# theo2021/OnDA

Hardware: AMD Instinct MI355X
Metric: adaptation-step images/sec (fwd+bwd+proto) 512x1024 bs=4 (higher is better)
Workload: dtype f32 (f16x2 split emulation); 1 GPU; hybrid_switch adaptation step (step + update_ema), 1024x512, bs=4 per micro-batch, 1 micro-batch(es) per GPU and optimizer step, dynamic branch, DeepLabV2-ResNet50 ProDA head, random-init weights; global_batch=4, parallelism=dp1, branch=dynamic, micro_batches_per_gpu=1, inputs=resident in HBM

## Files before the change

### include/onda_hip.h

```cpp
#ifndef ONDA_HIP_H
#define ONDA_HIP_H

#include <stdint.h>

#ifdef __cplusplus
extern "C" {
#endif

typedef void* onda_stream_t;

#define ONDA_OK 0
#define ONDA_EINVAL (-1)
#define ONDA_EALIGN (-2)

typedef struct OndaConv {
  int B, Hi, Wi, Cin;
  int Ho, Wo, Cout;
  int kh, kw, stride, dil, pad;
  int ldx;
  int ldy;
  int ldr;
  int out_os;
  int Hf, Wf;
  int relu;
// ... 89 lines not shown

typedef struct OndaBnSide {
  const float* x;
  const float* partials;
  int tiles, tile_rows;
  float *mean, *invstd, *xhat_amax;
  float *running_mean, *running_var;
  int64_t* nbt;
  float momentum;
  const float *gamma, *beta;
  void* dx;
  float* dx_amax;
} OndaBnSide;
int onda_bn_pair_fwd_l2(const OndaBnSide* a, const OndaBnSide* b, float eps, int relu, void* out, float* out_amax, int64_t M, int C,
                        uint8_t* relu_mask, int64_t split, int run_group, onda_stream_t s);
int64_t onda_bn_pair_bwd_l2_ws(int64_t M, int C);
int onda_bn_pair_bwd_l2(const float* dout, const uint8_t* relu_mask, const OndaBnSide* a, const OndaBnSide* b, float* ws, int64_t M,
                        int C, int relu, int64_t split, onda_stream_t s);
int onda_bn_pair_bwd_affine_l2(const float* dout, const uint8_t* relu_mask, const OndaBnSide* a, const OndaBnSide* b, float* ws,
                               int64_t M, int C, int relu, int64_t split, float* dgamma_a, float* dbeta_a, float* dgamma_b,
                               float* dbeta_b, onda_stream_t s);

int onda_conv_wgrad_l2_variant(int Cout, int Cin);
int64_t onda_conv2d_wgrad_l2_table_stride(const OndaConv* c);
int onda_conv2d_wgrad_l2_table(const OndaConv* c, int32_t* table, onda_stream_t s);
int onda_conv2d_wgrad_l2(const void* xl, int64_t xplane, const float* xamax, const void* dyl, int64_t dyplane, const float* dyamax,
                         float* slabs, int lddy, int splitk, const OndaConv* c, onda_stream_t s);

int onda_conv2d_wgrad(const float* x, const float* dy, float* slabs, int lddy, int splitk,
                      const OndaConv* c, onda_stream_t s);
int onda_wgrad_reduce(const float* slabs, float* dw, int splitk, int Cout, int taps, int Cin,
                      int Cout_real, int Cin_real, int flat_k, int accumulate, onda_stream_t s);

int onda_pack_weight_fwd(const float* w_oihw, float* dst, int Cout, int Cin, int taps, int Cout_pad, int Kp,
                         onda_stream_t s);
int onda_pack_weight_dgrad(const float* w_oihw, float* dst, int Cout, int Cin, int taps, int Cout_pad,
                           onda_stream_t s);

int onda_stem_im2col(const float* x_nchw, float* col, int B, int H, int W, int Ho, int Wo, int Kp, onda_stream_t s);

int onda_bn_finalize(const float* partials, int tiles, int C, int64_t count, float eps, float* mean, float* invstd,
                     float* running_mean, float* running_var, int64_t* num_batches_tracked, float momentum,
                     onda_stream_t s);
int onda_bn_stats(const float* x, int64_t M, int C, int ldx, float* partials, int* tiles_out, onda_stream_t s);
int onda_bn_apply(const float* x, const float* mean, const float* invstd, const float* gamma, const float* beta,
                  const float* residual, float* out, int64_t M, int C, int relu, float* amax, onda_stream_t s);
// ... 154 lines not shown
```

### onda_amd/_lib.py

```python
import ctypes
import os
from ctypes import POINTER, Structure, c_char_p, c_float, c_int, c_int64, c_void_p

HERE = os.path.dirname(os.path.abspath(__file__))
LIB_PATH = os.environ.get("ONDA_LIB_PATH") or os.path.join(HERE, "libonda_hip.so")

P = c_void_p
I, L, F = c_int, c_int64, c_float


class OndaConv(Structure):
    _fields_ = [(n, c_int) for n in ("B Hi Wi Cin Ho Wo Cout kh kw stride dil pad ldx ldy ldr out_os Hf Wf relu").split()] + \
               [("run_if", c_void_p), ("stat_split", c_int64), ("plain_schedule", c_int), ("pix_table", c_void_p),
                ("pix_stride", c_int64)]


class OndaSwitchCfg(Structure):
    _fields_ = [("limit", c_int), ("level_kind", c_int), ("use_exp", c_int), ("pad_", c_int), ("exp_const", ctypes.c_double),
                ("one_minus_exp_const", ctypes.c_double), ("taps_total", ctypes.c_double), ("gray_lo", ctypes.c_double),
                ("gray_hi", ctypes.c_double), ("dev_threshold", ctypes.c_double)]


class OndaLimbOut(Structure):
    _fields_ = [("out", c_void_p), ("out_plane", c_int64), ("out_bound", c_void_p), ("out_amax", c_void_p), ("kb", c_void_p),
# ... 41 lines not shown
    "onda_conv2d_fwd": (I, [P, P, P, P, P, P, P, P, POINTER(OndaConv), P]),
    "onda_absmax": (I, [P, L, I, I, P, P]),
    "onda_pack_weight_h2": (I, [P, P, I, I, I, I, I, I, I, P, P]),
    "onda_pack_weights_h2_multi": (I, [P, I, L, P]),
    "onda_pack_blocks": (I, [I, I, I]),
    "onda_split_h2": (I, [P, L, I, I, P, I, L, P, P]),
    "onda_stem_im2col_l2": (I, [P, P, P, L, I, I, I, I, I, I, P]),
    "onda_s2d_split_h2": (I, [P, I, I, I, I, I, I, F, P, P, P]),
    "onda_d2s_bwd": (I, [P, P, P, I, I, I, I, I, I, F, P, P, P]),
    "onda_debug_stamps": (None, [P]),
    "onda_conv2d_fwd_l2_limbs": (I, [P, L, P, P, P, P, P, P, P, P, P]),
    "onda_switch_state_doubles": (I, [I]),
    "onda_switch_max_window": (I, []),
    "onda_switch_step": (I, [P, P, P, I, P, POINTER(OndaSwitchCfg), P, P]),
    "onda_select_prior": (I, [P, P, F, P, F, P, L, P]),
    "onda_gate_scalar": (I, [P, P, P, P]),
    "onda_conv_l2_variant": (I, [L, I]),
    "onda_conv_l2_kernel_id": (I, [L, I, I, I]),
    "onda_conv_l2_tiles_m": (I, [L, I, I, I]),
    "onda_conv_l2_tiles_m_split": (I, [L, I, I, I, L, I, POINTER(c_int)]),
    "onda_conv_l2_live_fraction": (ctypes.c_double, [POINTER(OndaConv), I]),
    "onda_conv_wgrad_l2_live_fraction": (ctypes.c_double, [POINTER(OndaConv), I]),
    "onda_conv_wgrad_l2_variant": (I, [I, I]),
    "onda_conv2d_wgrad_l2_table_stride": (L, [POINTER(OndaConv)]),
    "onda_conv2d_wgrad_l2_table": (I, [POINTER(OndaConv), P, P]),
    "onda_conv2d_wgrad_l2": (I, [P, L, P, P, L, P, P, I, I, POINTER(OndaConv), P]),
    "onda_conv2d_fwd_l2": (I, [P, L, P, P, P, P, P, P, P, P, I, P, P, POINTER(OndaConv), P]),
    "onda_conv2d_taps_fwd_l2": (I, [P, P, P, P, P, P, P, P, P, P, P, POINTER(OndaConv), POINTER(c_int), I, P]),
    "onda_pack_sum_h2": (I, [POINTER(c_void_p), I, P, P, I, I, I, I, I, P, P]),
    "onda_bn_finalize_l2": (I, [P, I, I, L, F, P, P, P, P, P, F, P, P, P, I, P, P, L, I, I, P, I, P]),
    "onda_bn_apply_l2": (I, [P, P, P, P, P, P, L, P, P, L, P, L, I, I, P, L, P]),
    "onda_bn_bwd_l2_ws": (L, [L, I]),
    "onda_bn_train_l2": (I, [P, P, I, F, P, P, P, P, P, F, P, P, P, P, I, P, P, P, L, I, P, L, I, I, P]),
    "onda_bn_bwd_l2": (I, [P, P, L, P, P, P, P, P, P, L, P, P, P, L, I, I, P, L, I, P]),
    "onda_bn_bwd_affine_l2": (I, [P, P, L, P, P, P, P, P, P, L, P, P, P, L, I, I, P, L, I, P, P, P]),
    "onda_bn_pair_fwd_l2": (I, [POINTER(OndaBnSide), POINTER(OndaBnSide), F, I, P, P, L, I, P, L, I, P]),
    "onda_bn_pair_bwd_l2_ws": (L, [L, I]),
    "onda_bn_pair_bwd_l2": (I, [P, P, POINTER(OndaBnSide), POINTER(OndaBnSide), P, L, I, I, L, P]),
    "onda_bn_pair_bwd_affine_l2": (I, [P, P, POINTER(OndaBnSide), POINTER(OndaBnSide), P, L, I, I, L, P, P, P, P, P]),
    "onda_conv2d_wgrad": (I, [P, P, P, I, I, POINTER(OndaConv), P]),
    "onda_wgrad_reduce": (I, [P, P, I, I, I, I, I, I, I, I, P]),
    "onda_pack_weight_fwd": (I, [P, P, I, I, I, I, I, P]),
    "onda_pack_weight_dgrad": (I, [P, P, I, I, I, I, P]),
    "onda_stem_im2col": (I, [P, P, I, I, I, I, I, I, P]),
    "onda_bn_finalize": (I, [P, I, I, L, F, P, P, P, P, P, F, P]),
    "onda_bn_stats": (I, [P, L, I, I, P, POINTER(c_int), P]),
# ... 99 lines not shown
```

### onda_amd/csrc/conv_common.h

```cpp
#pragma once
#include "common.h"

struct ConvK {
  const float* x;
  const void* w;
  float* y;
  const float* scale;
  const float* shift;
  const float* res;
  float* stats;
  OndaConv c;
  int M, tilesM, tilesN, taps, kcper;
  float* ws;
  int tiles_dp;
  float* amax = nullptr;
  int skip_dead_taps = 1;
  int late_issue = 1;
  _Float16* yl = nullptr;
  long long yplane = 0;
  float* ybound = nullptr;
  const float* kb = nullptr;
  const float* xtrue = nullptr;
  const _Float16* resl = nullptr;
  long long resplane = 0;
  const float* res_amax = nullptr;
  const float* res_true = nullptr;
  unsigned long long* stamps = nullptr;
  int stats_rows = 2;
  long long x_total = 0;
};

struct WgradK {
  const float* x;
  const float* dy;
  float* slabs;
  OndaConv c;
  int M, lddy, splitk, mchunk, tilesN, tilesC, taps;
  long long x_total = 0, dy_total = 0;
  unsigned long long* stamps = nullptr;
  const int* pix = nullptr;
  long long pix_stride = 0;
};

constexpr int BK = 32;

template <class B>
__device__ __forceinline__ int xcd_band(B bid, int nblk) {
  const int q = nblk >> 3, r = nblk & 7, xcd = bid & 7;
  return (xcd < r ? xcd * (q + 1) : r * (q + 1) + (xcd - r) * q) + (bid >> 3);
}

struct SkItem {
  bool dp;
  int tile, k_begin, k_end;
};
struct SkTile {
  long long t0, t1;
};
struct StreamK {
  int KT, tiles_dp, G;
// ... 167 lines not shown
```

### onda_amd/csrc/conv_l2.hip

```cpp
#include "conv_common.h"
#include "limbs.h"

namespace {

typedef _Float16 f16x8 __attribute__((ext_vector_type(8)));
typedef _Float16 f16x4 __attribute__((ext_vector_type(4)));
typedef int i32x4 __attribute__((ext_vector_type(4)));

#define ZZ(i, jj) (((i) & 1) ? 3 - (jj) : (jj))

#define MFMA_SNAKE(MI, ACC, A, B)                                                                                       \
  _Pragma("unroll") for (int i = 0; i < (MI); ++i) _Pragma("unroll") for (int jj = 0; jj < 4; ++jj)                     \
      ACC[i][ZZ(i, jj)] = __builtin_amdgcn_mfma_f32_16x16x32_f16(A, B[ZZ(i, jj)], ACC[i][ZZ(i, jj)], 0, 0, 0)
#define FRAG_READ4(DST, P) \
  _Pragma("unroll") for (int j = 0; j < 4; ++j) DST = *reinterpret_cast<const f16x8*>((P) + j * 2048)
template <int MI>
__device__ __forceinline__ void acc_clear(f32x4 (&acc)[MI][4], f32x4 (&accx)[MI][4]) {
#pragma unroll
  for (int i = 0; i < MI; ++i)
#pragma unroll
    for (int j = 0; j < 4; ++j)
#pragma unroll
      for (int e = 0; e < 4; ++e) acc[i][j][e] = accx[i][j][e] = 0.f;
}
// ... 1296 lines not shown
      }
      *reinterpret_cast<f32x4*>(srow) = s1;
      *reinterpret_cast<f32x4*>(srow + c.Cout) = s2;
      if (SR == 4) {
        *reinterpret_cast<f32x4*>(srow + 2 * c.Cout) = mn;
        *reinterpret_cast<f32x4*>(srow + 3 * c.Cout) = mxv;
      }
    }
  }
}

template <int OFS = 0>
__device__ __forceinline__ f16x8 tr_read8(unsigned a0, unsigned a1) {
  u32x2 lo, hi;
  asm volatile("ds_read_b64_tr_b16 %0, %1 offset:%2" : "=v"(lo) : "v"(a0), "n"(OFS));
  asm volatile("ds_read_b64_tr_b16 %0, %1 offset:%2" : "=v"(hi) : "v"(a1), "n"(OFS));
  const u32x4 r = {lo[0], lo[1], hi[0], hi[1]};
  return __builtin_bit_cast(f16x8, r);
}
__device__ __forceinline__ void lds_wait(f16x8& a, f16x8& b, f16x8& c_, f16x8& d) {
  asm volatile("s_waitcnt lgkmcnt(0)" : "+v"(a), "+v"(b), "+v"(c_), "+v"(d));
}

template <int WM, int WN, int STAGES, int OCC, int MODE = 0>
__global__ __launch_bounds__(WM * WN * 64, OCC) void conv_wgrad_l2_kernel(const WgradK a, unsigned xplane, unsigned dyplane, unsigned x_bytes,
                                                                         unsigned dy_bytes, const float* __restrict__ xamax,
                                                                         const float* __restrict__ dyamax) {
  constexpr int NW = WM * WN;
  constexpr int SA = (64 * WM) / 128, SB = (64 * WN) / 128;
  static_assert(SA >= 1 && SB >= 1, "tiles are multiples of 128 channels");
  constexpr int SUB = 32 * 512;
  constexpr int A_BYTES = SA * SUB, STAGE = A_BYTES + SB * SUB;
  constexpr int GPW = 8 / NW;
  static_assert(GPW >= 1 && 8 % NW == 0, "8 pixel groups per K-step");
  constexpr int DPW = GPW * (SA + SB) * 2;
  constexpr bool STAGGER = NW == 8;
  constexpr int MAX_KT = 2048;
  __shared__ __attribute__((aligned(16))) unsigned char lds[STAGES * STAGE + MAX_KT * 2];

  const OndaConv& c = a.c;
  const int t = threadIdx.x, lane = t & 63, wave = __builtin_amdgcn_readfirstlane(t >> 6);
  const int wm = wave / WN, wn = wave % WN;
  const bool late = wave >= NW / 2;

  int bid = xcd_band(blockIdx.x, gridDim.x);
  const int tile_c = bid % a.tilesC;
  bid /= a.tilesC;
  const int tap = bid % a.taps;
  bid /= a.taps;
  const int tile_n = bid % a.tilesN;
  const int ks = bid / a.tilesN;
  const int n0 = tile_n * (64 * WM), c0 = tile_c * (64 * WN);
  const int mbeg = ks * a.mchunk;
  const int mend = min(a.M, mbeg + a.mchunk);
  const int KT = mend > mbeg ? (mend - mbeg + 31) / 32 : 0;
  const int rr = tap / c.kw, ss = tap - rr * c.kw;
  const int dh = rr * c.dil - c.pad, dw = ss * c.dil - c.pad;
  unsigned long long* stp = a.stamps != nullptr && t == 0 && blockIdx.x < 4096 ? a.stamps + (size_t)blockIdx.x * 8 : nullptr;
  if (stp) stp[0] = __builtin_amdgcn_s_memtime();
  constexpr unsigned PAST = 0x7FFFF000u;
  const int b_first = mbeg / (c.Ho * c.Wo);
  const long long x_at = (long long)b_first * c.Hi * c.Wi * c.ldx * 4, dy_at = (long long)mbeg * a.lddy * 4;
  const long long x_left = a.x_total - x_at;
  const long long dy_left = MODE == 1 ? (long long)(mend - mbeg) * a.lddy * 4 : a.dy_total - dy_at;
  const __amdgpu_buffer_rsrc_t rx = make_rsrc(reinterpret_cast<const char*>(a.x) + x_at, (unsigned)(x_left < PAST ? (x_left > 0 ? x_left : 0) : PAST));
  const __amdgpu_buffer_rsrc_t rdy = make_rsrc(reinterpret_cast<const char*>(a.dy) + dy_at, (unsigned)(dy_left < PAST ? (dy_left > 0 ? dy_left : 0) : PAST));
  const Scale2 sx = scale_of(xamax), sd = scale_of(dyamax);
  const float unscale_a = sx.inv, unscale_b = sd.inv;

  unsigned short* live_list = reinterpret_cast<unsigned short*>(lds + STAGES * STAGE);
  int nlive = 0;
  {
    unsigned char* flags = lds;
    for (int kt = t; kt < KT; kt += NW * 64) {
      const int m_first = mbeg + kt * 32, m_last = min(mend, m_first + 32) - 1;
      const int r_first = m_first / c.Wo, r_last = m_last / c.Wo;
      bool live = false;
      for (int r = r_first; r <= r_last; ++r) live |= (unsigned)((r % c.Ho) * c.stride + dh) < (unsigned)c.Hi;
      flags[kt] = live;
    }
    __syncthreads();
    for (int base = 0; base < KT; base += 64) {
      const bool f = base + lane < KT && flags[base + lane];
      const unsigned long long mask = __ballot(f);
      if (f) live_list[nlive + __popcll(mask & ((1ull << lane) - 1))] = (unsigned short)(base + lane);
      nlive += __popcll(mask);
    }
    __syncthreads();
  }
  auto live_at = [&](int i) -> int { return __builtin_amdgcn_readfirstlane((int)live_list[i]); };

  const int lam = lane >> 5, limb = (lane >> 4) & 1;
  unsigned ch_dy[GPW][2][SA], ch_x[GPW][2][SB];
#pragma unroll
  for (int d = 0; d < GPW; ++d)
#pragma unroll
    for (int h = 0; h < 2; ++h) {
      const int row = (wave * GPW + d) * 4 + 2 * h + lam;
      const int swz = ((row & 3) << 2) | ((row >> 2) & 3);
      const int ch = (lane & 15) ^ swz;
#pragma unroll
      for (int sI = 0; sI < SA; ++sI) {
        const int n = n0 + sI * 128 + ch * 8;
        ch_dy[d][h][sI] = n < c.Cout ? (unsigned)(limb_at(0, n, 0) + limb * LIMB2_OFS) * 2u : PAST;
      }
#pragma unroll
      for (int sI = 0; sI < SB; ++sI) {
        const int cc = c0 + sI * 128 + ch * 8;
        ch_x[d][h][sI] = cc < c.Cin ? (unsigned)(limb_at(0, cc, 0) + limb * LIMB2_OFS) * 2u : PAST;
      }
    }
  int p_m[GPW], p_wo[GPW], p_ho[GPW], p_b[GPW];
#pragma unroll
  for (int d = 0; d < GPW; ++d) {
    const int m = mbeg + (wave * GPW + d) * 4 + 2 * lam;
    p_m[d] = m;
    p_wo[d] = m % c.Wo;
    const int tq = m / c.Wo;
    p_ho[d] = tq % c.Ho;
    p_b[d] = tq / c.Ho - b_first;
  }
  int k_decoded = 0;
  unsigned pdy_s[GPW][2], px_s[GPW][2];
  int stage_s = 0;
  auto issue_part = [&](int h) {
#if defined(__HIP_DEVICE_COMPILE__)
#pragma unroll
    for (int d = 0; d < GPW; ++d) {
      const int grp = wave * GPW + d;
#pragma unroll
      for (int sI = 0; sI < SA; ++sI) {
        unsigned char* dst = lds + stage_s + sI * SUB + (grp * 2 + h) * 1024;
        const unsigned vo = pdy_s[d][h] + ch_dy[d][h][sI];
        __builtin_amdgcn_raw_ptr_buffer_load_lds(rdy, (__attribute__((address_space(3))) void*)dst, 16, vo, 0, 0, 0);
      }
#pragma unroll
      for (int sI = 0; sI < SB; ++sI) {
        unsigned char* dst = lds + stage_s + A_BYTES + sI * SUB + (grp * 2 + h) * 1024;
        const unsigned vo = px_s[d][h] + ch_x[d][h][sI];
        __builtin_amdgcn_raw_ptr_buffer_load_lds(rx, (__attribute__((address_space(3))) void*)dst, 16, vo, 0, 0, 0);
      }
    }
#else
    (void)h;
#endif
  };
  auto issue_addr = [&](int kt, int stage_off) {
    stage_s = stage_off;
    const int adv = (kt - k_decoded) * 32;
    k_decoded = kt;
#pragma unroll
    for (int d = 0; d < GPW; ++d) {
      p_m[d] += adv;
      p_wo[d] += adv;
      while (p_wo[d] >= c.Wo) {
        p_wo[d] -= c.Wo;
        if (++p_ho[d] == c.Ho) {
          p_ho[d] = 0;
          ++p_b[d];
        }
      }
      int m = p_m[d], wo = p_wo[d], ho = p_ho[d], b = p_b[d];
#pragma unroll
      for (int h = 0; h < 2; ++h) {
        unsigned pdy = OOB, px = OOB;
        if (m < mend) {
          pdy = (unsigned)(m - mbeg) * (unsigned)a.lddy * 4u;
          const int hi = ho * c.stride + dh, wi = wo * c.stride + dw;
          if ((unsigned)hi < (unsigned)c.Hi && (unsigned)wi < (unsigned)c.Wi) px = (unsigned)(((b * c.Hi + hi) * c.Wi + wi) * c.ldx) * 4u;
        }
        pdy_s[d][h] = pdy;
        px_s[d][h] = px;
        ++m;
        if (++wo == c.Wo) {
          wo = 0;
          if (++ho == c.Ho) {
            ho = 0;
            ++b;
          }
        }
      }
    }
  };
  auto issue = [&](int kt, int stage_off) {
    issue_addr(kt, stage_off);
    issue_part(0);
    issue_part(1);
  };

  unsigned fa[4][2], fb[4][2];
  {
    const int g = lane >> 4, q = (lane >> 2) & 3, pp = lane & 3;
#pragma unroll
    for (int h = 0; h < 2; ++h) {
      const int row = 8 * g + 4 * h + q;
      const int swz = ((row & 3) << 2) | ((row >> 2) & 3);
#pragma unroll
      for (int i = 0; i < 4; ++i) {
        const int cha = (wm & 1) * 8 + 2 * i + (pp >> 1), chb = (wn & 1) * 8 + 2 * i + (pp >> 1);
        fa[i][h] = (unsigned)((wm >> 1) * SUB + 512 * row + 16 * (cha ^ swz) + 8 * (pp & 1));
        fb[i][h] = (unsigned)(A_BYTES + (wn >> 1) * SUB + 512 * row + 16 * (chb ^ swz) + 8 * (pp & 1));
        asm volatile("" : "+v"(fa[i][h]), "+v"(fb[i][h]));
      }
    }
  }

  f32x4 acc[4][4], accx[4][4];
  acc_clear(acc, accx);
// ... 17 lines not shown
      issue_part(0);
      st_issue = st_issue + STAGE == STAGES * STAGE ? 0 : st_issue + STAGE;
      ++i_iss;
    }
  };
  auto issue_second_part = [&]() {
    if (second_part_due) issue_part(1);
    second_part_due = false;
  };
  auto wait_landed_half = [&](bool first_part_in_flight) {
    if (first_part_in_flight)
      asm volatile("s_waitcnt vmcnt(%0)" ::"n"(DPW / 2) : "memory");
    else
      asm volatile("s_waitcnt vmcnt(0)" ::: "memory");
  };
  auto wait_landed = [&](bool more_in_flight) {
    if (more_in_flight)
      asm volatile("s_waitcnt vmcnt(%0)" ::"n"(DPW) : "memory");
    else
      asm volatile("s_waitcnt vmcnt(0)" ::: "memory");
  };
  constexpr int AHEAD = STAGES >= 3 ? 2 : 1;
  static_assert(!STAGGER || STAGES >= 3, "the staggered halves need two steps in flight");
  if constexpr (MODE == 0) {
    if (i_iss < nlive) issue_next();
    if (AHEAD == 2 && i_iss < nlive) issue_next();
  }
  f16x8 af[4][2], bf[4], b1[4];
  const unsigned lds0 = (unsigned)(size_t)(__attribute__((address_space(3))) unsigned char*)lds;
  unsigned base;
  auto prepare = [&]() {
    base = lds0 + st_read;
    st_read = st_read + STAGE == STAGES * STAGE ? 0 : st_read + STAGE;
#pragma unroll
    for (int i = 0; i < 4; ++i) {
      const unsigned a0 = base + fa[i][0], a1 = base + fa[i][1];
      af[i][0] = tr_read8<0>(a0, a1);
      af[i][1] = tr_read8<256>(a0, a1);
    }
#pragma unroll
    for (int j = 0; j < 4; ++j) {
      const unsigned a0 = base + fb[j][0], a1 = base + fb[j][1];
      bf[j] = tr_read8<256>(a0, a1);
      if constexpr (STAGGER) b1[j] = tr_read8<0>(a0, a1);
    }
  };
  auto prepared = [&]() {
    lds_wait(af[0][0], af[1][0], af[2][0], af[3][0]);
    lds_wait(af[0][1], af[1][1], af[2][1], af[3][1]);
    lds_wait(bf[0], bf[1], bf[2], bf[3]);
    if constexpr (STAGGER) lds_wait(b1[0], b1[1], b1[2], b1[3]);
    __builtin_amdgcn_sched_barrier(0);
  };
  auto compute = [&]() {
    if constexpr (!STAGGER) {
#pragma unroll
      for (int j = 0; j < 4; ++j) b1[j] = tr_read8(base + fb[j][0], base + fb[j][1]);
    }
    MFMA_SNAKE(4, accx, af[i][0], bf);
    if constexpr (!STAGGER) lds_wait(b1[0], b1[1], b1[2], b1[3]);
    if constexpr (STAGGER) issue_second_part();
    __builtin_amdgcn_sched_barrier(0);
    MFMA_SNAKE(4, accx, af[i][1], b1);
    MFMA_SNAKE(4, acc, af[i][0], b1);
  };
  if constexpr (MODE >= 1) {
    static_assert(STAGGER && GPW == 1 && STAGES == 3, "the eight-wave tile");
    const unsigned lddy4 = (unsigned)a.lddy * 4u, ldx4 = (unsigned)c.ldx * 4u;
    unsigned dy_lane[2], x_lane[2];
#pragma unroll
    for (int h = 0; h < 2; ++h) {
      const unsigned pix = (unsigned)(wave * 4 + 2 * lam + h);
      dy_lane[h] = pix * lddy4;
      x_lane[h] = (pix + (unsigned)(mbeg - b_first * c.Ho * c.Wo)) * ldx4;
    }
    const int base_px = b_first * c.Hi * c.Wi;
    const i32x4* tab = MODE == 2 ? reinterpret_cast<const i32x4*>(a.pix + (size_t)tap * a.pix_stride + mbeg + wave * 4) : nullptr;
    i32x4 t_next = {-1, -1, -1, -1};
    auto offsets = [&](int kt, const i32x4& te, unsigned kill) {
#pragma unroll
      for (int h = 0; h < 2; ++h) {
        pdy_s[0][h] = (unsigned)kt * 32u * lddy4 + dy_lane[h] + kill;
        if constexpr (MODE == 1) {
          px_s[0][h] = (unsigned)kt * 32u * ldx4 + x_lane[h] + kill;
        } else {
          const int lo = te[h], hi = te[2 + h];
          const int e = lam ? hi : lo;
          px_s[0][h] = (e >= 0 ? __umul24((unsigned)(e - base_px), ldx4) : PAST) + kill;
        }
// ... 61 lines not shown
        __builtin_amdgcn_sched_group_barrier(0x008, 16, 0);
#pragma unroll
        for (int q = 0; q < 14; ++q) {
          __builtin_amdgcn_sched_group_barrier(0x008, 1, 0);
          __builtin_amdgcn_sched_group_barrier(0x002, 2, 0);
        }
#pragma unroll
        for (int q = 0; q < NI; ++q) {
          __builtin_amdgcn_sched_group_barrier(0x008, 2, 0);
          __builtin_amdgcn_sched_group_barrier(0x006, 2, 0);
          __builtin_amdgcn_sched_group_barrier(0x020, 1, 0);
        }
        __builtin_amdgcn_sched_group_barrier(0x008, 48 - 16 - 14 - 2 * NI, 0);
        __builtin_amdgcn_sched_barrier(0);
        entry_wait(t_after);
        kt_next = kt_after;
        t_next = t_after;
      }
      if (!late) __builtin_amdgcn_s_barrier();
      asm volatile("s_waitcnt vmcnt(0)" ::: "memory");
    }
  } else if constexpr (!STAGGER) {
    for (; i_cur < nlive; ++i_cur) {
      wait_landed(AHEAD == 2 && i_cur + 1 < nlive);
      __builtin_amdgcn_s_barrier();
      if (i_iss < nlive) issue_next();
      prepare();
      prepared();
      compute();
    }
  } else {
    if (late && nlive > 0) {
      wait_landed(nlive > 1);
      __builtin_amdgcn_s_barrier();
    }
    for (; i_cur < nlive; ++i_cur) {
      if (!late) wait_landed(i_cur + 1 < nlive);
      __builtin_amdgcn_s_barrier();
      unsigned long long tk0 = 0, tk1 = 0, tk2 = 0;
      if (stp) tk0 = __builtin_amdgcn_s_memtime();
      issue_first_part();
      if (stp) tk1 = __builtin_amdgcn_s_memtime();
      prepare();
      prepared();
      if (stp) tk2 = __builtin_amdgcn_s_memtime();
      if (late && i_cur + 1 < nlive) wait_landed_half(i_cur + 2 < nlive);
      __builtin_amdgcn_s_barrier();
      if (stp && i_cur == nlive / 2) {
        const unsigned long long tk3 = __builtin_amdgcn_s_memtime();
        stp[4] = ((tk1 - tk0) << 40) | ((tk2 - tk1) << 20) | (tk3 - tk2);
        stp[6] = tk3;
      }
      compute();
      if (stp && i_cur == nlive / 2) stp[7] = __builtin_amdgcn_s_memtime() - stp[6];
    }
    if (!late && nlive > 0) __builtin_amdgcn_s_barrier();
  }

#pragma unroll
  for (int i = 0; i < 4; ++i)
#pragma unroll
    for (int j = 0; j < 4; ++j) acc[i][j] = unscale2(limb_fold(acc[i][j], accx[i][j]), unscale_a, unscale_b);
  if (stp) stp[2] = __builtin_amdgcn_s_memtime();
  __syncthreads();
  float* tr = reinterpret_cast<float*>(lds + (t >> 6) * 4096);
  const int cl = (lane & 15) * 4, rl = lane >> 4;
  const int cc = c0 + wn * 64 + cl;
#pragma unroll
  for (int i = 0; i < 4; ++i) {
#pragma unroll
    for (int jn = 0; jn < 4; ++jn)
#pragma unroll
      for (int e = 0; e < 4; ++e) tr[(4 * (lane >> 4) + e) * 64 + jn * 16 + (lane & 15)] = acc[i][jn][e];
    __builtin_amdgcn_wave_barrier();
#pragma unroll
    for (int r = 0; r < 4; ++r) {
      const int row = 4 * r + rl;
      const f32x4 v = *reinterpret_cast<const f32x4*>(tr + row * 64 + cl);
      const int n = n0 + (wm * 4 + i) * 16 + row;
      if (n < c.Cout && cc < c.Cin) *reinterpret_cast<f32x4*>(a.slabs + (((size_t)ks * c.Cout + n) * a.taps + tap) * c.Cin + cc) = v;
    }
    __builtin_amdgcn_wave_barrier();
  }
  if (stp) stp[3] = __builtin_amdgcn_s_memtime();
}

}

extern "C" {

int onda_split_h2(const float* x, int64_t rows, int C, int ldx, void* dst, int ldo, int64_t plane, const float* amax,
                  onda_stream_t s) {
  (void)plane;
  ONDA_REQUIRE(x && dst && amax && rows > 0 && C > 0 && C % 8 == 0 && ldx >= C && ldx % 4 == 0 && ldo >= C && ldo % 32 == 0);
  if (!ONDA_ALIGNED16(x) || !ONDA_ALIGNED16(dst)) return ONDA_EALIGN;
  const long long n = rows * (C / 8);
  const int blocks = (int)(n / 256 / 4 + 1 > 2048 ? 2048 : n / 256 / 4 + 1);
  hipLaunchKernelGGL(split_h2_kernel, dim3(blocks), dim3(256), 0, ONDA_STREAM(s), x, (long long)rows, C, ldx,
                     static_cast<_Float16*>(dst), ldo, (long long)plane, amax);
  return ONDA_LAUNCH_RESULT();
}

int onda_stem_im2col_l2(const float* x_nchw, const float* xamax, void* dst, int64_t plane, int B, int H, int W, int Ho, int Wo,
// ... 101 lines not shown
  for (int tile_m = 0; tile_m * q.tilesN < tiles_dp; ++tile_m) {
    const int n_dp = tiles_dp - tile_m * q.tilesN < q.tilesN ? tiles_dp - tile_m * q.tilesN : q.tilesN;
    const long long m0 = (long long)tile_m * q.BM, m_last = (M < m0 + q.BM ? M : m0 + q.BM) - 1;
    const long long r0 = m0 / c->Wo, r1 = m_last / c->Wo;
    int live = 0;
    for (int tp = 0; tp < taps; ++tp) {
      const int dh = (tp / c->kw) * c->dil - c->pad;
      bool alive = false;
      for (long long r = r0; r <= r1 && !alive; ++r) alive = (unsigned)((int)(r % c->Ho) * c->stride + dh) < (unsigned)c->Hi;
      live += alive;
    }
    if (live == 0) live = 1;
    live_steps += (long long)n_dp * live * kcper;
  }
  return (double)live_steps / ((double)tiles * taps * kcper);
}

double onda_conv_wgrad_l2_live_fraction(const OndaConv* c, int splitk) {
  if (!c || splitk < 1) return 1.0;
  const long long M = (long long)c->B * c->Ho * c->Wo;
  const int taps = c->kh * c->kw;
  if (M <= 0 || taps <= 1) return 1.0;
  const long long mchunk = ((M + splitk - 1) / splitk + 31) / 32 * 32;
  long long live = 0, all = 0;
  for (int ks = 0; ks < splitk; ++ks) {
    const long long mbeg = ks * mchunk, mend = M < mbeg + mchunk ? M : mbeg + mchunk;
    const long long KT = mend > mbeg ? (mend - mbeg + 31) / 32 : 0;
    all += KT * taps;
    for (int tp = 0; tp < taps; ++tp) {
      const int dh = (tp / c->kw) * c->dil - c->pad;
      for (long long kt = 0; kt < KT; ++kt) {
        const long long m_first = mbeg + kt * 32, m_last = (mend < m_first + 32 ? mend : m_first + 32) - 1;
        bool alive = false;
        for (long long r = m_first / c->Wo; r <= m_last / c->Wo && !alive; ++r)
          alive = (unsigned)((int)(r % c->Ho) * c->stride + dh) < (unsigned)c->Hi;
        live += alive;
      }
    }
  }
  return all > 0 ? (double)live / (double)all : 1.0;
}

static int l2_fwd_impl(const void* xl, int64_t xplane, const float* xamax, const void* w2, const float* wamax, float* y,
                       const float* scale, const float* shift, const float* residual, float* stats, int stats_rows, float* ws,
                       float* yamax, const OndaConv* c, onda_stream_t s, const OndaLimbOut* lo, const TapTable* tab = nullptr) {
  ONDA_REQUIRE(xl && xamax && w2 && wamax && (y || lo) && c && ws && (stats_rows == 2 || stats_rows == 4));
  if (lo != nullptr) {
    ONDA_REQUIRE(lo->out && lo->out_bound && lo->kb && lo->xtrue && !stats && !residual);
    ONDA_REQUIRE(c->out_os == 1 && c->Hf == c->Ho && c->Wf == c->Wo && c->ldy % 32 == 0 && c->ldy >= c->Cout);
    ONDA_REQUIRE(!lo->res || (lo->res_amax && c->ldr % 32 == 0 && c->ldr >= c->Cout));
    if (!ONDA_ALIGNED16(lo->out) || (lo->res && !ONDA_ALIGNED16(lo->res))) return ONDA_EALIGN;
  }
  ONDA_REQUIRE(c->Cin > 0 && c->Cin % 32 == 0 && c->Cout > 0 && c->Cout % 4 == 0 && c->ldx % 32 == 0 && c->ldx >= c->Cin);
  ONDA_REQUIRE(c->kh >= 1 && c->kw >= 1 && c->stride >= 1 && c->dil >= 1 && c->out_os >= 1);
  (void)xplane;
  if (!ONDA_ALIGNED16(xl) || !ONDA_ALIGNED16(w2)) return ONDA_EALIGN;
  if (c->ldy % 4 != 0 || (y && !ONDA_ALIGNED16(y)) || (residual && (c->ldr % 4 != 0 || !ONDA_ALIGNED16(residual)))) return ONDA_EALIGN;
  if (scale && !ONDA_ALIGNED16(scale)) return ONDA_EALIGN;
  if (shift && !ONDA_ALIGNED16(shift)) return ONDA_EALIGN;
// ... 147 lines not shown
  TapTable tab;
  for (int t = 0; t < TAPS_MAX; ++t) {
    const int dh = t < ntaps ? taps[2 * t] : 0, dw = t < ntaps ? taps[2 * t + 1] : 0;
    ONDA_REQUIRE(dh > -16384 && dh < 16384 && dw > -16384 && dw < 16384);
    tab.d[t] = (int)((unsigned)(dh & 0xFFFF) | ((unsigned)dw << 16));
  }
  OndaConv g = *c;
  g.kh = 1;
  g.kw = ntaps;
  g.dil = 1;
  g.pad = 0;
  g.stat_split = 0;
  return l2_fwd_impl(xl, 0, xamax, w2, wamax, y, nullptr, shift, residual, nullptr, 2, ws, yamax, &g, s, nullptr, &tab);
}

static unsigned long long* g_debug_stamps = nullptr;
void onda_debug_stamps(void* p) { g_debug_stamps = static_cast<unsigned long long*>(p); }

int onda_conv_wgrad_l2_variant(int Cout, int Cin) {
  (void)Cin;
  return Cout >= 256 ? 0 : 1;
}

}

namespace {
__global__ __launch_bounds__(256) void wgrad_pixel_table_kernel(int* __restrict__ t, long long stride, int B, int Hi, int Wi, int Ho,
                                                               int Wo, int kw, int cstride, int dil, int pad) {
  const long long M = (long long)B * Ho * Wo;
  const int tap = blockIdx.y, rr = tap / kw, ss = tap - rr * kw;
  for (long long m = (long long)blockIdx.x * 256 + threadIdx.x; m < stride; m += (long long)gridDim.x * 256) {
    int v = -1;
    if (m < M) {
      const int wo = (int)(m % Wo);
      const long long q = m / Wo;
      const int ho = (int)(q % Ho), b = (int)(q / Ho);
      const int hi = ho * cstride + rr * dil - pad, wi = wo * cstride + ss * dil - pad;
      if ((unsigned)hi < (unsigned)Hi && (unsigned)wi < (unsigned)Wi) v = (b * Hi + hi) * Wi + wi;
    }
    t[(size_t)tap * stride + m] = v;
  }
}
}

extern "C" {

// ... 32 lines not shown
  const long long M = (long long)c->B * c->Ho * c->Wo;
  ONDA_REQUIRE(M > 0 && M < (1ll << 31));
  const long long x_total = (long long)c->B * c->Hi * c->Wi * c->ldx * 4;
  const long long dy_total = M * lddy * 4;
  WgradK k;
  k.x = static_cast<const float*>(xl); k.dy = static_cast<const float*>(dyl); k.slabs = slabs; k.c = *c;
  k.M = (int)M;
  k.lddy = lddy;
  k.splitk = splitk;
  k.stamps = g_debug_stamps;
  k.mchunk = (int)(((M + splitk - 1) / splitk + 31) / 32 * 32);
  ONDA_REQUIRE(k.mchunk / 32 <= 2048);
  {
    const long long img = (long long)c->Hi * c->Wi * c->ldx * 4, per_wg = k.mchunk / ((long long)c->Ho * c->Wo) + 2;
    ONDA_REQUIRE((long long)k.mchunk * lddy * 4 < 0x7FFFF000ll && (per_wg < c->B ? per_wg : c->B) * img < 0x7FFFF000ll);
  }
  k.x_total = x_total;
  k.dy_total = dy_total;
  k.taps = c->kh * c->kw;
  const int variant = onda_conv_wgrad_l2_variant(c->Cout, c->Cin);
  const int TN = variant == 0 ? 256 : 128;
  k.tilesN = (c->Cout + TN - 1) / TN;
  k.tilesC = (c->Cin + 127) / 128;
  const unsigned grid = (unsigned)(k.tilesN * k.tilesC * k.taps * splitk);
  const unsigned xpl = 0, dypl = 0;
  static const int mode = getenv("ONDA_WGRAD_MODE") ? atoi(getenv("ONDA_WGRAD_MODE")) : 1;
  const bool linear = wgrad_l2_linear(c);
  if (variant == 0 && mode == 1 && linear)
    hipLaunchKernelGGL((conv_wgrad_l2_kernel<4, 2, 3, 2, 1>), dim3(grid), dim3(512), 0, ONDA_STREAM(s), k, xpl, dypl, 0u, 0u, xamax, dyamax);
  else if (variant == 0 && mode == 1 && c->pix_table != nullptr && (k.pix = c->pix_table, k.pix_stride = c->pix_stride, true))
    hipLaunchKernelGGL((conv_wgrad_l2_kernel<4, 2, 3, 2, 2>), dim3(grid), dim3(512), 0, ONDA_STREAM(s), k, xpl, dypl, 0u, 0u, xamax, dyamax);
  else if (variant == 0)
    hipLaunchKernelGGL((conv_wgrad_l2_kernel<4, 2, 3, 2>), dim3(grid), dim3(512), 0, ONDA_STREAM(s), k, xpl, dypl, 0u, 0u, xamax, dyamax);
  else
    hipLaunchKernelGGL((conv_wgrad_l2_kernel<2, 2, 2, 2>), dim3(grid), dim3(256), 0, ONDA_STREAM(s), k, xpl, dypl, 0u, 0u, xamax, dyamax);
  return ONDA_LAUNCH_RESULT();
}

}
```

### onda_amd/ops/conv.py

```python
import ctypes
from ctypes import byref

import torch

from .. import _lib
from .._lib import OndaLimbOut, call, query
from . import _state
from ._state import STEM_K
from .core import _conv_ws, _desc, _group_split, _l2_name, _launch, _p, _require_cuda, _stream, as_nhwc, conv_out_size, nhwc_ld
from .limbs import H2Weight, Limbs, amax_slot, is_limb_only, known_amax, limb_only, limbs_of, tag_amax
from .tables import _table


def _use_l2(wp, cin):
    return isinstance(wp, H2Weight) and _state.H2_PATH == "dma" and cin % 32 == 0


def _pack_h2(weight, rows_pad, kp, dgrad, cout_pad):
    cout, cin, kh, kw = weight.shape
    w = weight.detach().contiguous()
    slot = known_amax(weight)
    if slot is None:
        slot = amax_slot(weight.device, long_lived=True)
        call("onda_absmax", _p(w), 1, w.numel(), w.numel(), _p(slot), _stream())
# ... 168 lines not shown
            raise RuntimeError("onda_amd: strided data gradient is implemented for 1x1 convs only")
        dx = torch.zeros(B, Hi, Wi, cin, device=dy.device, dtype=torch.float32)
        d = _desc(B, Ho, Wo, Co, Ho, Wo, cin, 1, 1, 1, 0, ldy, cin, out_os=stride, Hf=Hi, Wf=Wi)
    if _use_l2(wpd, Co):
        dyl = limbs_of(dy)
        d.ldx = dyl.ld
        _launch_l2("dgrad", dyl, wpd, dx, d, yamax=yamax, tag_dims=(B * Ho * Wo if stride != 1 else B * Hi * Wi, cin, Co, k, stride, dil))
        return dx
    if yamax is not None:
        raise RuntimeError("onda_amd: max|dx| from the data gradient's epilogue needs the pre-split path")
    if is_limb_only(dy):
        raise RuntimeError("onda_amd: a limb-only gradient reached a data-gradient kernel that does not take limb planes")
    if isinstance(wpd, H2Weight):
        raise RuntimeError("onda_amd: a pre-split weight reached a data gradient the pre-split kernels do not take (Cout % 32 != 0)")
    _launch("conv_fwd_kernel<128,%d>" % (128 if cin > 64 else 64), 2.0 * B * Ho * Wo * cin * k * k * Co, "onda_conv2d_fwd",
            _p(dy), _p(wpd), _p(dx), None, None, None, None, _p(_conv_ws(dy.device)), byref(d), _stream(),
            tag=("dgrad", B * Ho * Wo if stride != 1 else B * Hi * Wi, cin, Co, k, stride, dil))
    return dx


def _wgrad_splitk(M, cout, cin, taps, l2=False):
    if l2:
        tn = 256 if query("onda_conv_wgrad_l2_variant", cout, cin) == 0 else 128
        tiles = -(-cout // tn) * -(-cin // 128) * taps
        G = query("onda_conv_ws_floats") // (3 * 128 * 128) // (2 if tn == 256 else 1)
        return max(_best_splitk(M, cout, cin, taps, tiles, G, 3.2e14 if tn == 256 else 2.0e14), -(-M // 65536))
    t = 128 if (cout > 64 and cin > 64) else 64
    tiles = -(-cout // t) * -(-cin // t) * taps
    G = query("onda_conv_ws_floats") // (3 * 128 * 128) * (1 if t == 128 else 2)
    return _best_splitk(M, cout, cin, taps, tiles, G, 1.2e14)


def _best_splitk(M, cout, cin, taps, tiles, G, rate):
    t_ideal = 2.0 * M * cout * cin * taps / rate
    wbytes = 4.0 * cout * cin * taps
    best, best_t = 1, None
    for sk in range(1, 257):
        if sk > 1 and (M // sk < 256 or sk * wbytes > (512 << 20)):
            break
        blocks = tiles * sk
        eff = (blocks / G) / -(-blocks // G)
        est = t_ideal / eff + 2.0 * sk * wbytes / 3e12
        if best_t is None or est < best_t * 0.995:
            best, best_t = sk, est
    return best


# ... 426 lines not shown
```

Before: 43.84 images/s.

## Group two taps per wgrad block for small-Cin convs and add single-row address mode

For weight-gradient convs with Cin<=64 on the 4-wave variant, each block now handles two filter taps, one per wave column, so a 128-wide channel tile is not half wasted and each dy tile is loaded once for both taps. A new MODE 3 path computes one pixel address per lane and distributes it with ds_bpermute, which is meant to cut per-step address arithmetic, and it becomes the default for the variant-1 kernel. The split-k heuristic and live-fraction estimator account for the grouped taps. The cost is more kernel template instances and more complex liveness and store-bounds logic.

```diff
diff --git a/include/onda_hip.h b/include/onda_hip.h
--- a/include/onda_hip.h
+++ b/include/onda_hip.h
@@ -135,6 +135,7 @@
                                float* dbeta_b, onda_stream_t s);
 
 int onda_conv_wgrad_l2_variant(int Cout, int Cin);
+int onda_conv_wgrad_l2_tap_groups(int Cout, int Cin, int taps);
 int64_t onda_conv2d_wgrad_l2_table_stride(const OndaConv* c);
 int onda_conv2d_wgrad_l2_table(const OndaConv* c, int32_t* table, onda_stream_t s);
 int onda_conv2d_wgrad_l2(const void* xl, int64_t xplane, const float* xamax, const void* dyl, int64_t dyplane, const float* dyamax,
diff --git a/onda_amd/_lib.py b/onda_amd/_lib.py
--- a/onda_amd/_lib.py
+++ b/onda_amd/_lib.py
@@ -87,6 +87,7 @@
     "onda_conv_l2_live_fraction": (ctypes.c_double, [POINTER(OndaConv), I]),
     "onda_conv_wgrad_l2_live_fraction": (ctypes.c_double, [POINTER(OndaConv), I]),
     "onda_conv_wgrad_l2_variant": (I, [I, I]),
+    "onda_conv_wgrad_l2_tap_groups": (I, [I, I, I]),
     "onda_conv2d_wgrad_l2_table_stride": (L, [POINTER(OndaConv)]),
     "onda_conv2d_wgrad_l2_table": (I, [POINTER(OndaConv), P, P]),
     "onda_conv2d_wgrad_l2": (I, [P, L, P, P, L, P, P, I, I, POINTER(OndaConv), P]),
diff --git a/onda_amd/csrc/conv_common.h b/onda_amd/csrc/conv_common.h
--- a/onda_amd/csrc/conv_common.h
+++ b/onda_amd/csrc/conv_common.h
@@ -36,6 +36,7 @@
   float* slabs;
   OndaConv c;
   int M, lddy, splitk, mchunk, tilesN, tilesC, taps;
+  int tap_groups = 0;
   long long x_total = 0, dy_total = 0;
   unsigned long long* stamps = nullptr;
   const int* pix = nullptr;
diff --git a/onda_amd/csrc/conv_l2.hip b/onda_amd/csrc/conv_l2.hip
--- a/onda_amd/csrc/conv_l2.hip
+++ b/onda_amd/csrc/conv_l2.hip
@@ -1342,7 +1342,7 @@
   asm volatile("s_waitcnt lgkmcnt(0)" : "+v"(a), "+v"(b), "+v"(c_), "+v"(d));
 }
 
-template <int WM, int WN, int STAGES, int OCC, int MODE = 0>
+template <int WM, int WN, int STAGES, int OCC, int MODE = 0, int TG = 1>
 __global__ __launch_bounds__(WM * WN * 64, OCC) void conv_wgrad_l2_kernel(const WgradK a, unsigned xplane, unsigned dyplane, unsigned x_bytes,
                                                                          unsigned dy_bytes, const float* __restrict__ xamax,
                                                                          const float* __restrict__ dyamax) {
@@ -1353,6 +1353,8 @@
   constexpr int A_BYTES = SA * SUB, STAGE = A_BYTES + SB * SUB;
   constexpr int GPW = 8 / NW;
   static_assert(GPW >= 1 && 8 % NW == 0, "8 pixel groups per K-step");
+  static_assert(TG == 1 || (TG == 2 && WN == 2 && (MODE == 0 || MODE == 3)), "tap groups: one x sub-image, a wave column per tap");
+  static_assert(MODE != 3 || (NW == 4 && SA == 1 && SB == 1), "MODE 3 is the four-wave tile's");
   constexpr int DPW = GPW * (SA + SB) * 2;
   constexpr bool STAGGER = NW == 8;
   constexpr int MAX_KT = 2048;
@@ -1366,8 +1368,9 @@
   int bid = xcd_band(blockIdx.x, gridDim.x);
   const int tile_c = bid % a.tilesC;
   bid /= a.tilesC;
-  const int tap = bid % a.taps;
-  bid /= a.taps;
+  const int ncol = TG == 1 ? a.taps : a.tap_groups;
+  const int tap = (bid % ncol) * TG;
+  bid /= ncol;
   const int tile_n = bid % a.tilesN;
   const int ks = bid / a.tilesN;
   const int n0 = tile_n * (64 * WM), c0 = tile_c * (64 * WN);
@@ -1376,13 +1379,16 @@
   const int KT = mend > mbeg ? (mend - mbeg + 31) / 32 : 0;
   const int rr = tap / c.kw, ss = tap - rr * c.kw;
   const int dh = rr * c.dil - c.pad, dw = ss * c.dil - c.pad;
+  const bool tap1 = TG == 2 && tap + 1 < a.taps;
+  const int rr1 = TG == 2 ? (tap + 1) / c.kw : rr, ss1 = TG == 2 ? tap + 1 - rr1 * c.kw : ss;
+  const int dh1 = rr1 * c.dil - c.pad, dw1 = ss1 * c.dil - c.pad;
   unsigned long long* stp = a.stamps != nullptr && t == 0 && blockIdx.x < 4096 ? a.stamps + (size_t)blockIdx.x * 8 : nullptr;
   if (stp) stp[0] = __builtin_amdgcn_s_memtime();
   constexpr unsigned PAST = 0x7FFFF000u;
   const int b_first = mbeg / (c.Ho * c.Wo);
   const long long x_at = (long long)b_first * c.Hi * c.Wi * c.ldx * 4, dy_at = (long long)mbeg * a.lddy * 4;
   const long long x_left = a.x_total - x_at;
-  const long long dy_left = MODE == 1 ? (long long)(mend - mbeg) * a.lddy * 4 : a.dy_total - dy_at;
+  const long long dy_left = MODE == 1 || MODE == 3 ? (long long)(mend - mbeg) * a.lddy * 4 : a.dy_total - dy_at;
   const __amdgpu_buffer_rsrc_t rx = make_rsrc(reinterpret_cast<const char*>(a.x) + x_at, (unsigned)(x_left < PAST ? (x_left > 0 ? x_left : 0) : PAST));
   const __amdgpu_buffer_rsrc_t rdy = make_rsrc(reinterpret_cast<const char*>(a.dy) + dy_at, (unsigned)(dy_left < PAST ? (dy_left > 0 ? dy_left : 0) : PAST));
   const Scale2 sx = scale_of(xamax), sd = scale_of(dyamax);
@@ -1396,7 +1402,10 @@
       const int m_first = mbeg + kt * 32, m_last = min(mend, m_first + 32) - 1;
       const int r_first = m_first / c.Wo, r_last = m_last / c.Wo;
       bool live = false;
-      for (int r = r_first; r <= r_last; ++r) live |= (unsigned)((r % c.Ho) * c.stride + dh) < (unsigned)c.Hi;
+      for (int r = r_first; r <= r_last; ++r) {
+        live |= (unsigned)((r % c.Ho) * c.stride + dh) < (unsigned)c.Hi;
+        if constexpr (TG == 2) live |= tap1 && (unsigned)((r % c.Ho) * c.stride + dh1) < (unsigned)c.Hi;
+      }
       flags[kt] = live;
     }
     __syncthreads();
@@ -1426,10 +1435,18 @@
       }
 #pragma unroll
       for (int sI = 0; sI < SB; ++sI) {
-        const int cc = c0 + sI * 128 + ch * 8;
-        ch_x[d][h][sI] = cc < c.Cin ? (unsigned)(limb_at(0, cc, 0) + limb * LIMB2_OFS) * 2u : PAST;
-      }
-    }
+        const int cc = TG == 2 ? (ch & 7) * 8 : c0 + sI * 128 + ch * 8;
+        const bool there = cc < c.Cin && (TG == 1 || ch < 8 || tap1);
+        ch_x[d][h][sI] = there ? (unsigned)(limb_at(0, cc, 0) + limb * LIMB2_OFS) * 2u : PAST;
+      }
+    }
+  int dh_l[2], dw_l[2];
+#pragma unroll
+  for (int h = 0; h < 2; ++h) {
+    const bool second = TG == 2 && (((lane >> 3) & 1) ^ h) != 0;
+    dh_l[h] = second ? dh1 : dh;
+    dw_l[h] = second ? dw1 : dw;
+  }
   int p_m[GPW], p_wo[GPW], p_ho[GPW], p_b[GPW];
 #pragma unroll
   for (int d = 0; d < GPW; ++d) {
@@ -1441,6 +1458,26 @@
     p_b[d] = tq / c.Ho - b_first;
   }
   int k_decoded = 0;
+  int q_m = 0, q_wo = 0, q_ho = 0, q_b = 0, q_dh = dh, q_dw = dw;
+  unsigned dyc[GPW][2], src_x[GPW][2];
+  if constexpr (MODE == 3) {
+    const int m = mbeg + wave * (4 * GPW) + (lane & 7);
+    q_m = m;
+    q_wo = m % c.Wo;
+    const int tq = m / c.Wo;
+    q_ho = tq % c.Ho;
+    q_b = tq / c.Ho - b_first;
+    if (TG == 2 && (lane & 8) != 0) q_dh = dh1, q_dw = dw1;
+#pragma unroll
+    for (int d = 0; d < GPW; ++d)
+#pragma unroll
+      for (int h = 0; h < 2; ++h) {
+        const int pix = 4 * d + 2 * lam + h;
+        dyc[d][h] = (unsigned)(wave * (4 * GPW) + pix) * (unsigned)a.lddy * 4u + ch_dy[d][h][0];
+        const bool second = TG == 2 && (((lane >> 3) & 1) ^ h) != 0;
+        src_x[d][h] = 4u * (unsigned)(pix + (second ? 8 : 0));
+      }
+  }
   unsigned pdy_s[GPW][2], px_s[GPW][2];
   int stage_s = 0;
   auto issue_part = [&](int h) {
@@ -1451,7 +1488,7 @@
 #pragma unroll
       for (int sI = 0; sI < SA; ++sI) {
         unsigned char* dst = lds + stage_s + sI * SUB + (grp * 2 + h) * 1024;
-        const unsigned vo = pdy_s[d][h] + ch_dy[d][h][sI];
+        const unsigned vo = MODE == 3 ? pdy_s[d][h] : pdy_s[d][h] + ch_dy[d][h][sI];
         __builtin_amdgcn_raw_ptr_buffer_load_lds(rdy, (__attribute__((address_space(3))) void*)dst, 16, vo, 0, 0, 0);
       }
 #pragma unroll
@@ -1486,7 +1523,7 @@
         unsigned pdy = OOB, px = OOB;
         if (m < mend) {
           pdy = (unsigned)(m - mbeg) * (unsigned)a.lddy * 4u;
-          const int hi = ho * c.stride + dh, wi = wo * c.stride + dw;
+          const int hi = ho * c.stride + (TG == 2 ? dh_l[h] : dh), wi = wo * c.stride + (TG == 2 ? dw_l[h] : dw);
           if ((unsigned)hi < (unsigned)c.Hi && (unsigned)wi < (unsigned)c.Wi) px = (unsigned)(((b * c.Hi + hi) * c.Wi + wi) * c.ldx) * 4u;
         }
         pdy_s[d][h] = pdy;
@@ -1502,8 +1539,38 @@
       }
     }
   };
+  auto issue_addr_one = [&](int kt, int stage_off) {
+#if defined(__HIP_DEVICE_COMPILE__)
+    stage_s = stage_off;
+    const int adv = (kt - k_decoded) * 32;
+    k_decoded = kt;
+    q_m += adv;
+    q_wo += adv;
+    while (q_wo >= c.Wo) {
+      q_wo -= c.Wo;
+      if (++q_ho == c.Ho) {
+        q_ho = 0;
+        ++q_b;
+      }
+    }
+    unsigned px = OOB;
+    const int hi = q_ho * c.stride + q_dh, wi = q_wo * c.stride + q_dw;
+    if (q_m < mend && (unsigned)hi < (unsigned)c.Hi && (unsigned)wi < (unsigned)c.Wi) px = (unsigned)(((q_b * c.Hi + hi) * c.Wi + wi) * c.ldx) * 4u;
+    const unsigned dyk = (unsigned)kt * 32u * (unsigned)a.lddy * 4u;
+#pragma unroll
+    for (int d = 0; d < GPW; ++d)
+#pragma unroll
+      for (int h = 0; h < 2; ++h) {
+        pdy_s[d][h] = dyk + dyc[d][h];
+        px_s[d][h] = (unsigned)__builtin_amdgcn_ds_bpermute((int)src_x[d][h], (int)px);
+      }
+#else
+    (void)kt, (void)stage_off;
+#endif
+  };
   auto issue = [&](int kt, int stage_off) {
-    issue_addr(kt, stage_off);
+    if constexpr (MODE == 3) issue_addr_one(kt, stage_off);
+    else issue_addr(kt, stage_off);
     issue_part(0);
     issue_part(1);
   };
@@ -1567,7 +1634,7 @@
   };
   constexpr int AHEAD = STAGES >= 3 ? 2 : 1;
   static_assert(!STAGGER || STAGES >= 3, "the staggered halves need two steps in flight");
-  if constexpr (MODE == 0) {
+  if constexpr (MODE == 0 || MODE == 3) {
     if (i_iss < nlive) issue_next();
     if (AHEAD == 2 && i_iss < nlive) issue_next();
   }
@@ -1609,7 +1676,7 @@
     MFMA_SNAKE(4, accx, af[i][1], b1);
     MFMA_SNAKE(4, acc, af[i][0], b1);
   };
-  if constexpr (MODE >= 1) {
+  if constexpr (MODE == 1 || MODE == 2) {
     static_assert(STAGGER && GPW == 1 && STAGES == 3, "the eight-wave tile");
     const unsigned lddy4 = (unsigned)a.lddy * 4u, ldx4 = (unsigned)c.ldx * 4u;
     unsigned dy_lane[2], x_lane[2];
@@ -1717,12 +1784,31 @@
     }
   } else if constexpr (!STAGGER) {
     for (; i_cur < nlive; ++i_cur) {
+#if defined(ONDA_WGRAD_SLOT_STAMPS)
+      const bool stamp = stp && i_cur == nlive / 2;
+      unsigned long long tk0 = 0, tk1 = 0, tk2 = 0, tk3 = 0;
+      if (stamp) tk0 = __builtin_amdgcn_s_memtime();
+      wait_landed(AHEAD == 2 && i_cur + 1 < nlive);
+      __builtin_amdgcn_s_barrier();
+      if (stamp) tk1 = __builtin_amdgcn_s_memtime();
+      if (i_iss < nlive) issue_next();
+      if (stamp) tk2 = __builtin_amdgcn_s_memtime();
+      prepare();
+      prepared();
+      if (stamp) tk3 = __builtin_amdgcn_s_memtime();
+      compute();
+      if (stamp) {
+        stp[4] = ((tk2 - tk1) << 40) | ((tk3 - tk2) << 20) | (tk1 - tk0);
+        stp[7] = __builtin_amdgcn_s_memtime() - tk3;
+      }
+#else
       wait_landed(AHEAD == 2 && i_cur + 1 < nlive);
       __builtin_amdgcn_s_barrier();
       if (i_iss < nlive) issue_next();
       prepare();
       prepared();
       compute();
+#endif
     }
   } else {
     if (late && nlive > 0) {
@@ -1760,7 +1846,8 @@
   __syncthreads();
   float* tr = reinterpret_cast<float*>(lds + (t >> 6) * 4096);
   const int cl = (lane & 15) * 4, rl = lane >> 4;
-  const int cc = c0 + wn * 64 + cl;
+  const int cc = TG == 2 ? cl : c0 + wn * 64 + cl;
+  const int tap_st = TG == 2 ? tap + wn : tap;
 #pragma unroll
   for (int i = 0; i < 4; ++i) {
 #pragma unroll
@@ -1773,7 +1860,8 @@
       const int row = 4 * r + rl;
       const f32x4 v = *reinterpret_cast<const f32x4*>(tr + row * 64 + cl);
       const int n = n0 + (wm * 4 + i) * 16 + row;
-      if (n < c.Cout && cc < c.Cin) *reinterpret_cast<f32x4*>(a.slabs + (((size_t)ks * c.Cout + n) * a.taps + tap) * c.Cin + cc) = v;
+      if (n < c.Cout && cc < c.Cin && tap_st < a.taps)
+        *reinterpret_cast<f32x4*>(a.slabs + (((size_t)ks * c.Cout + n) * a.taps + tap_st) * c.Cin + cc) = v;
     }
     __builtin_amdgcn_wave_barrier();
   }
@@ -1921,19 +2009,23 @@
   const int taps = c->kh * c->kw;
   if (M <= 0 || taps <= 1) return 1.0;
   const long long mchunk = ((M + splitk - 1) / splitk + 31) / 32 * 32;
+  const int tg = onda_conv_wgrad_l2_tap_groups(c->Cout, c->Cin, taps) != taps ? 2 : 1;
   long long live = 0, all = 0;
   for (int ks = 0; ks < splitk; ++ks) {
     const long long mbeg = ks * mchunk, mend = M < mbeg + mchunk ? M : mbeg + mchunk;
     const long long KT = mend > mbeg ? (mend - mbeg + 31) / 32 : 0;
     all += KT * taps;
-    for (int tp = 0; tp < taps; ++tp) {
-      const int dh = (tp / c->kw) * c->dil - c->pad;
+    for (int tp = 0; tp < taps; tp += tg) {
+      const int n_tp = tp + tg <= taps ? tg : taps - tp;
       for (long long kt = 0; kt < KT; ++kt) {
         const long long m_first = mbeg + kt * 32, m_last = (mend < m_first + 32 ? mend : m_first + 32) - 1;
         bool alive = false;
-        for (long long r = m_first / c->Wo; r <= m_last / c->Wo && !alive; ++r)
-          alive = (unsigned)((int)(r % c->Ho) * c->stride + dh) < (unsigned)c->Hi;
-        live += alive;
+        for (int u = tp; u < tp + n_tp && !alive; ++u) {
+          const int dh = (u / c->kw) * c->dil - c->pad;
+          for (long long r = m_first / c->Wo; r <= m_last / c->Wo && !alive; ++r)
+            alive = (unsigned)((int)(r % c->Ho) * c->stride + dh) < (unsigned)c->Hi;
+        }
+        live += alive ? n_tp : 0;
       }
     }
   }
@@ -2127,6 +2219,12 @@
   return Cout >= 256 ? 0 : 1;
 }
 
+int onda_conv_wgrad_l2_tap_groups(int Cout, int Cin, int taps) {
+  const char* e = getenv("ONDA_WGRAD_TAP_GROUPS");
+  const bool on = e == nullptr || atoi(e) != 0;
+  return on && taps > 1 && Cin <= 64 && onda_conv_wgrad_l2_variant(Cout, Cin) == 1 ? (taps + 1) / 2 : taps;
+}
+
 }
 
 namespace {
@@ -2205,9 +2303,11 @@
   const int TN = variant == 0 ? 256 : 128;
   k.tilesN = (c->Cout + TN - 1) / TN;
   k.tilesC = (c->Cin + 127) / 128;
-  const unsigned grid = (unsigned)(k.tilesN * k.tilesC * k.taps * splitk);
+  k.tap_groups = onda_conv_wgrad_l2_tap_groups(c->Cout, c->Cin, k.taps);
+  const bool grouped = k.tap_groups != k.taps;
+  const unsigned grid = (unsigned)(k.tilesN * k.tilesC * k.tap_groups * splitk);
   const unsigned xpl = 0, dypl = 0;
-  static const int mode = getenv("ONDA_WGRAD_MODE") ? atoi(getenv("ONDA_WGRAD_MODE")) : 1;
+  const int mode = getenv("ONDA_WGRAD_MODE") ? atoi(getenv("ONDA_WGRAD_MODE")) : 1;
   const bool linear = wgrad_l2_linear(c);
   if (variant == 0 && mode == 1 && linear)
     hipLaunchKernelGGL((conv_wgrad_l2_kernel<4, 2, 3, 2, 1>), dim3(grid), dim3(512), 0, ONDA_STREAM(s), k, xpl, dypl, 0u, 0u, xamax, dyamax);
@@ -2215,6 +2315,12 @@
     hipLaunchKernelGGL((conv_wgrad_l2_kernel<4, 2, 3, 2, 2>), dim3(grid), dim3(512), 0, ONDA_STREAM(s), k, xpl, dypl, 0u, 0u, xamax, dyamax);
   else if (variant == 0)
     hipLaunchKernelGGL((conv_wgrad_l2_kernel<4, 2, 3, 2>), dim3(grid), dim3(512), 0, ONDA_STREAM(s), k, xpl, dypl, 0u, 0u, xamax, dyamax);
+  else if (grouped && mode == 1)
+    hipLaunchKernelGGL((conv_wgrad_l2_kernel<2, 2, 2, 2, 3, 2>), dim3(grid), dim3(256), 0, ONDA_STREAM(s), k, xpl, dypl, 0u, 0u, xamax, dyamax);
+  else if (mode == 1)
+    hipLaunchKernelGGL((conv_wgrad_l2_kernel<2, 2, 2, 2, 3>), dim3(grid), dim3(256), 0, ONDA_STREAM(s), k, xpl, dypl, 0u, 0u, xamax, dyamax);
+  else if (grouped)
+    hipLaunchKernelGGL((conv_wgrad_l2_kernel<2, 2, 2, 2, 0, 2>), dim3(grid), dim3(256), 0, ONDA_STREAM(s), k, xpl, dypl, 0u, 0u, xamax, dyamax);
   else
     hipLaunchKernelGGL((conv_wgrad_l2_kernel<2, 2, 2, 2>), dim3(grid), dim3(256), 0, ONDA_STREAM(s), k, xpl, dypl, 0u, 0u, xamax, dyamax);
   return ONDA_LAUNCH_RESULT();
diff --git a/onda_amd/ops/conv.py b/onda_amd/ops/conv.py
--- a/onda_amd/ops/conv.py
+++ b/onda_amd/ops/conv.py
@@ -214,7 +214,7 @@
 def _wgrad_splitk(M, cout, cin, taps, l2=False):
     if l2:
         tn = 256 if query("onda_conv_wgrad_l2_variant", cout, cin) == 0 else 128
-        tiles = -(-cout // tn) * -(-cin // 128) * taps
+        tiles = -(-cout // tn) * -(-cin // 128) * query("onda_conv_wgrad_l2_tap_groups", cout, cin, taps)
         G = query("onda_conv_ws_floats") // (3 * 128 * 128) // (2 if tn == 256 else 1)
         return max(_best_splitk(M, cout, cin, taps, tiles, G, 3.2e14 if tn == 256 else 2.0e14), -(-M // 65536))
     t = 128 if (cout > 64 and cin > 64) else 64
```

Result: no change. 43.95 images/s (median of 5 runs) (+0.2%).
